# ChristophReich1996/Multi-StyleGAN

Measured on AMD Instinct MI355X. Metric: training images/sec (G+D step, 256^2, seq=3x2ch), higher is better.
Workload: dtype bf16

## Files before the change

include/msg_hip.h:

```cpp
#ifndef MSG_HIP_H
#define MSG_HIP_H

#ifdef __cplusplus
extern "C" {
#endif

enum { MSG_OK = 0, MSG_EINVAL = -1, MSG_EUNSUPPORTED = -2, MSG_ELAUNCH = -3 };
enum { MSG_F32 = 0, MSG_BF16 = 1, MSG_F16 = 2, MSG_F64 = 3, MSG_F32_SPLIT = 4 };

#define MSG_ABI_VERSION 5
int msg_abi_version(void);
const char* msg_build_arch(void);
const char* msg_strerror(int code);

int msg_upfirdn2d(const void* x, const float* fir, void* y, int dtype,
                  int major, int in_h, int in_w, int minor, int kh, int kw,
                  int up_x, int up_y, int down_x, int down_y,
                  int pad_x0, int pad_x1, int pad_y0, int pad_y1, void* stream);

int msg_upfirdn2d_pitched(const void* x, const float* fir, void* y, int dtype,
                          int major, int in_h, int in_w, int minor, int in_pitch, int kh, int kw,
                          int up_x, int up_y, int down_x, int down_y,
                          int pad_x0, int pad_x1, int pad_y0, int pad_y1, void* stream);

// ... 18 lines not shown
                                     int noise_batch, float alpha, float scale, unsigned char* mask, void* stream);

int msg_fused_bias_act(const void* x, const float* bias, const void* ref, void* y, int dtype,
                       long long size_x, int step_b, int size_b,
                       const float* noise, const float* noise_weight, int noise_batch, int pix,
                       int act, int grad, float alpha, float scale, void* stream);

long long msg_bias_act_backward_workspace(long long size_x, int step_b, int size_b, int has_noise);
int msg_bias_act_backward(const void* gy, const void* out, void* gx, int dtype,
                          long long size_x, int step_b, int size_b,
                          float* grad_bias, const float* noise, float* grad_noise_weight,
                          int noise_batch, int pix, float alpha, float scale,
                          float* ws, long long ws_floats, void* stream);
int msg_channel_sums(const void* x, float* sums, int dtype, long long size_x, int C, float* ws, long long ws_floats,
                     void* stream);
int msg_bias_act_backward_mask(const void* gy, const unsigned char* mask, int tile_m, int tile_n, void* gx, int dtype,
                               long long size_x, int size_b,
                               float* grad_bias, const float* noise, float* grad_noise_weight,
                               int noise_batch, int pix, float alpha, float scale,
                               float* ws, long long ws_floats, void* stream);
int msg_sum_rows(const float* part, float* out, long long rows, int cols, void* stream);
int msg_bias_act_backward_mask_head(const void* gy, const void* ghead, const float* whead, const float* style,
                                    float wscale, int n_head, const unsigned char* mask, int tile_m, int tile_n,
                                    void* gx, int dtype, long long size_x, int size_b,
                                    float* grad_bias, const float* noise, float* grad_noise_weight,
                                    int noise_batch, int pix, float alpha, float scale,
                                    float* ws, long long ws_floats, void* stream);

int msg_conv2d_fprop(const void* x, const void* w, const float* bias, void* y, int dtype,
                     int B, int IH, int IW, int Cx, int Ck, int OH, int OW, int N, int ldy,
                     int kh, int kw, int stride, int pad, int in_up, int pixel_shuffle,
                     long long w_batch_stride, void* stream);
int msg_conv2d_wgrad(const void* gy, const void* x, float* gw, int dtype,
                     int B, int IH, int IW, int Cx, int I, int OH, int OW, int ldgy, int O, int ldgw,
                     int kh, int kw, int stride, int pad, int pixel_shuffle,
                     int per_sample, int k_chunks, int oi_major, float gain,
                     float* ws, long long ws_floats, void* stream);
long long msg_conv2d_wgrad_workspace(int dtype, int B, int IH, int IW, int Cx, int I, int OH, int OW, int ldgy,
                                     int O, int ldgw, int kh, int kw, int stride, int pad, int pixel_shuffle,
                                     int per_sample, int k_chunks);

int msg_demod_coeff(const float* W, const float* s, float* d, int B, int O, int I, int taps,
                    float scale, float eps, void* stream);
int msg_scale_rows_cols(const float* base, const float* rowscale, const float* colscale, void* out,
                        int dtype, int B, int R, int T, int C, int Ck, float gain, void* stream);
int msg_modulate_weights(const float* base, const float* wsq, const float* style, void* out, float* d_out,
                         int dtype, int B, int R, int O, int T, int C, int Ck, float scale, float eps, void* stream);
int msg_modulate_backward(const float* gwk, const float* W, const float* s, const float* d, float* gW,
                          float* gs_part, int B, int O, int I, int taps, int ldg, int o_group,
                          float scale, void* stream);
int msg_scale_rows_cols2(const float* base, const float* row1, const float* col1, const float* row2, const float* col2,
                         void* out, int dtype, int B, int R, int T, int C, int Ck, float gain, void* stream);
int msg_modulate_backward2(const float* gwk, const float* W, const float* s, const float* d, const float* v,
                           float* gW, float* gs_part, int B, int O, int I, int taps, int ldg, int o_group,
                           float scale, void* stream);

int msg_relayout_weight(const float* w, void* fwd, void* dgrad, float* wsq, int dtype,
                        int O, int I, int T, int Ck, int Ok, int flip, int t_major, float gain, void* stream);

int msg_gather_taps(const void* x, void* y, int dtype, int B, int H, int W, int Cx, int C, int kh, int kw,
                    int pad, int Ko, void* stream);
int msg_fold_taps(const void* g, const void* add, void* gx, int dtype, int B, int H, int W, int Ko, int C, int kh, int kw,
                  int pad, int ldx, int ld_add, void* stream);

int msg_scaled_add(const void* a, const void* b, void* y, int dtype, long long n, float beta, float gain, void* stream);
int msg_rgb_skip_merge(const void* conv, int dtype, int ld, const float* bias, const float* skip, const float* fir,
                       float* out, int B, int C, int H, int W, void* stream);
int msg_rgb_skip_merge_backward(const float* g, void* g_conv, int dtype, int ld, float* g_skip, const float* fir,
                                int B, int C, int H, int W, void* stream);
int msg_gamma_merge(const void* a, const void* b, const float* gamma, void* y, int dtype, long long n, float gain, void* stream);
long long msg_gamma_merge_backward_workspace(void);
int msg_gamma_merge_backward(const void* gy, const void* a, const float* gamma, void* ga, void* gb, float* g_gamma, int dtype,
                             long long n, float gain, float* ws, void* stream);
int msg_scaled_add_rows(const void* a, const void* b, void* y, int dtype, long long rows, int cols,
                        long long lda, long long ldb, long long ldy, float beta, float gain, void* stream);

int msg_softmax_rows(const void* x, void* y, int dtype, long long rows, int cols, void* stream);
int msg_softmax_rows_backward(const void* y, const void* gy, void* gx, int dtype, long long rows, int cols,
                              void* stream);
int msg_softmax_rows_backward2(const void* y, const void* gy, const void* v, void* d_y, void* d_gy, int dtype,
                               long long rows, int cols, void* stream);

int msg_nonlocal_attention_supported(int B, int Nq, int Nk, int dk, int dv);
int msg_nonlocal_attention_fwd(const void* q, const void* k, const void* vt, void* o, float* lse, int dtype,
                               int B, int Nq, int Nk, int dk, int dv, void* stream);
int msg_maxpool2x2_fwd(const void* x, void* y, unsigned short* idx, int dtype, int B, int H, int W, int C, long long ldx,
                       void* stream);
int msg_maxpool2x2_bwd(const void* gy, const unsigned short* idx, void* gx, int dtype, int B, int H, int W, int C,
                       void* stream);
int msg_maxpool2x2_gather(const void* v, const unsigned short* idx, void* out, int dtype, int B, int H, int W, int C,
                          long long ldv, void* stream);

int msg_nonlocal_attention_bwd_splits(int B, int Nq, int Nk);
int msg_nonlocal_attention_bwd(const void* q, const void* qt, const void* k, const void* kt, const void* v,
                               const void* dO, const void* dOt, const void* o, const float* lse, float* delta,
                               void* dq, void* dk_out, void* dv_out, float* workspace, int dtype,
                               int B, int Nq, int Nk, int dk, int dv, void* stream);

int msg_affine_warp(const float* x, float* y, const float* angle_deg, float angle_const, const float* scale_xy,
                    const float* select_u, const float* p, int rot_prob, float cx, float cy, int padding,
                    int align_corners, int B, int C, int H, int W, int backward, void* workspace, void* stream);

long long msg_minibatch_stddev_workspace(int C, int H, int W, int groups, int dtype);
int msg_minibatch_stddev(const void* x, void* y, float* stat, float* workspace, int dtype,
                         int B, int C, int H, int W, int ldx, int ldy, int groups, float alpha, void* stream);
int msg_minibatch_stddev_backward(const void* x, const void* gy, const float* gstat, void* gx, int dtype,
                                  int B, int C, int H, int W, int ldx, int ldgy, int ldgx, int groups,
                                  float alpha, void* stream);

int msg_conv2d_fprop_act(const void* x, const void* w, void* y, int dtype,
                         int B, int IH, int IW, int Cx, int Ck, int OH, int OW, int N, int ldy,
                         int kh, int kw, int stride, int pad, long long w_batch_stride,
                         const float* act_bias, const float* noise, const float* noise_weight,
                         int noise_batch, float alpha, float scale, void* stream);
int msg_conv2d_fprop_act_mask(const void* x, const void* w, void* y, int dtype,
                              int B, int IH, int IW, int Cx, int Ck, int OH, int OW, int N, int ldy,
                              int kh, int kw, int stride, int pad, long long w_batch_stride,
                              const float* act_bias, const float* noise, const float* noise_weight,
                              int noise_batch, float alpha, float scale, unsigned char* mask, void* stream);

int msg_conv2d_fprop_residual(const void* x, const void* w, void* y, int dtype,
                              int B, int IH, int IW, int Cx, int Ck, int OH, int OW, int N, int ldy,
                              int kh, int kw, int stride, int pad, long long w_batch_stride,
                              const void* residual, int res_ld, float gain, void* stream);

int msg_conv2d_fprop_act_backward(const void* x, const void* w, void* y, int dtype,
                                  int B, int IH, int IW, int Cx, int Ck, int OH, int OW, int N, int ldy,
                                  int kh, int kw, int stride, int pad, long long w_batch_stride,
                                  const void* residual, int res_ld,
                                  const unsigned char* sign_mask, int mask_tile_m, int mask_tile_n,
                                  const void* sign_map, int sign_ld, float alpha, float scale,
                                  float* grad_bias, const float* noise, int noise_batch, float* grad_noise_weight,
                                  float* ws, long long ws_floats, void* stream);

int msg_act_pointwise_head(const void* x, const float* bias, const float* w, float* y, int dtype,
                           long long npix, int C, float wscale, float alpha, float scale, void* stream);
long long msg_act_pointwise_head_backward_workspace(long long npix, int C);
int msg_act_pointwise_head_backward(const void* x, const float* bias, const float* w, const float* gy, void* gx,
                                    float* grad_bias_and_w, int dtype, long long npix, int C, float wscale,
                                    float alpha, float scale, float* ws, long long ws_floats, void* stream);

int msg_linear_fprop(const float* x, const float* w, const float* bias, float* y, int M, int N, int K,
                     float gain, float bias_gain, void* stream);
int msg_linear_dgrad(const float* gy, const float* w, float* gx, int M, int N, int K, float gain, void* stream);
int msg_linear_wgrad(const float* gy, const float* x, float* gw, float* gb, int M, int N, int K,
                     float gain, float bias_gain, void* stream);

int msg_linear_grouped_fprop(const float* x, const int* slot, const float* const* w, const float* const* bias, float* y,
                             int G, int M, int N, int K, int L, float gain, float bias_gain, void* stream);
int msg_linear_grouped_dgrad(const float* gy, const float* const* w, float* gx, int G, int M, int N, int K, float gain,
                             void* stream);
int msg_linear_grouped_wgrad(const float* gy, const float* x, const int* slot, float* gw, float* gb, int G, int M, int N,
                             int K, int L, float gain, float bias_gain, void* stream);
int msg_linear_grouped_wgrad_ptrs(const float* gy, const float* x, const int* slot, float* const* gw, float* const* gb, int G,
                                  int M, int N, int K, int L, float gain, float bias_gain, void* stream);

enum {
    MSG_PLAN_REG = 0,
    MSG_PLAN_DMA = 1,
    MSG_PLAN_PP = 2,
    MSG_PLAN_ROW3 = 3,
    MSG_PLAN_ROW3N = 4,
    MSG_PLAN_THIN = 5,
    MSG_PLAN_UPCONV = 6,
    MSG_FPLAN_FIELDS = 5
};
int msg_conv2d_fprop_launch_plan(int dtype, int B, int IH, int IW, int Cx, int Ck, int OH, int OW, int N, int ldy,
// ... 56 lines not shown
```

multi_stylegan_amd/csrc/attention.hip:

```cpp
#include "msg_common.h"
#include <stdlib.h>

typedef __bf16 bf16v8 __attribute__((ext_vector_type(8)));

namespace {

template <typename T> struct Mma;
template <> struct Mma<bf16_t> {
    typedef bf16v8 Frag;
    static constexpr int KS = 16;
    static constexpr int PAD = 8;
    static constexpr int VEC = 8;
    static __device__ __forceinline__ Frag load(const bf16_t* row, int s, int h) {
        return *reinterpret_cast<const Frag*>(row + 16 * s + 8 * h);
    }
    static __device__ __forceinline__ f32x16 mma(Frag a, Frag b, f32x16 c) {
        return __builtin_amdgcn_mfma_f32_32x32x16_bf16(a, b, c, 0, 0, 0);
    }
    static __device__ __forceinline__ float dot(Frag a, Frag b) {
        float acc = 0.f;
#pragma unroll
        for (int j = 0; j < 8; ++j) acc = fmaf((float)a[j], (float)b[j], acc);
        return acc;
    }
    static __device__ __forceinline__ void store4(bf16_t* p, float a, float b, float c, float d) {
        uint2 v;
        v.x = (uint32_t)f2bf(a) | ((uint32_t)f2bf(b) << 16);
        v.y = (uint32_t)f2bf(c) | ((uint32_t)f2bf(d) << 16);
        *reinterpret_cast<uint2*>(p) = v;
    }
    static __device__ __forceinline__ Frag load_t(const bf16_t* tile, int pitch, int col, int s, int lane) {
        typedef short s16x4 __attribute__((ext_vector_type(4)));
        typedef short s16x8 __attribute__((ext_vector_type(8)));
        const int g = lane >> 4, q = (lane >> 2) & 3, pq = lane & 3;
        const int kb = 8 * (g >> 1), cb = 16 * (g & 1);
        s16x4 part[2];
#pragma unroll
        for (int half = 0; half < 2; ++half) {
            const bf16_t* pa = tile + (16 * s + kb + 4 * half + q) * pitch + col + cb + 4 * pq;
            part[half] = __builtin_amdgcn_ds_read_tr16_b64_v4i16((s16x4 __attribute__((address_space(3)))*)(pa));
        }
        return __builtin_bit_cast(Frag, (s16x8)__builtin_shufflevector(part[0], part[1], 0, 1, 2, 3, 4, 5, 6, 7));
    }
};
template <> struct Mma<float> {
    typedef float Frag;
    static constexpr int KS = 2;
    static constexpr int PAD = 4;
    static constexpr int VEC = 4;
    static __device__ __forceinline__ Frag load(const float* row, int s, int h) { return row[2 * s + h]; }
    static __device__ __forceinline__ f32x16 mma(Frag a, Frag b, f32x16 c) {
        return __builtin_amdgcn_mfma_f32_32x32x2f32(a, b, c, 0, 0, 0);
    }
    static __device__ __forceinline__ float dot(Frag a, Frag b) { return a * b; }
    static __device__ __forceinline__ void store4(float* p, float a, float b, float c, float d) {
        *reinterpret_cast<float4*>(p) = make_float4(a, b, c, d);
    }
    static __device__ __forceinline__ Frag load_t(const float* tile, int pitch, int col, int s, int lane) {
        return tile[(2 * s + (lane >> 5)) * pitch + col + (lane & 31)];
    }
};

template <typename T, int ROWS, int COLS, bool PF, int THREADS = 256>
struct Stager {
    static constexpr int VEC = 16 / sizeof(T), CPR = COLS / VEC, TOTAL = ROWS * CPR, N = (TOTAL + THREADS - 1) / THREADS;
    static_assert(COLS % VEC == 0, "tile rows are whole 16-byte vectors");
    uint4 r[PF ? N : 1];
    const T* src;
    long long pitch;
    __device__ __forceinline__ void load(const T* g, long long g_pitch, int tid) {
        if constexpr (!PF) { src = g; pitch = g_pitch; return; }
#pragma unroll
        for (int i = 0; i < N; ++i) {
            const int c = tid + THREADS * i;
            if (TOTAL % THREADS == 0 || c < TOTAL) {
                const int row = c / CPR, cc = c - row * CPR;
                r[PF ? i : 0] = *reinterpret_cast<const uint4*>(g + row * g_pitch + cc * VEC);
            }
        }
    }
    __device__ __forceinline__ void store(T* lds, int l_pitch, int tid) const {
#pragma unroll
        for (int i = 0; i < N; ++i) {
            const int c = tid + THREADS * i;
            if (TOTAL % THREADS == 0 || c < TOTAL) {
                const int row = c / CPR, cc = c - row * CPR;
                *reinterpret_cast<uint4*>(lds + row * l_pitch + cc * VEC) =
                    PF ? r[PF ? i : 0] : *reinterpret_cast<const uint4*>(src + row * pitch + cc * VEC);
            }
        }
    }
};

__device__ __forceinline__ f32x16 zero16() {
    f32x16 z;
#pragma unroll
    for (int i = 0; i < 16; ++i) z[i] = 0.f;
    return z;
}

__device__ __forceinline__ void wave_lds_fence() { asm volatile("s_waitcnt lgkmcnt(0)" ::: "memory"); }

template <typename T, int DK, int DV, bool PF>
__global__ __launch_bounds__(256) void nl_attn_fwd_kernel(const T* __restrict__ q, const T* __restrict__ k,
                                                         const T* __restrict__ vt, T* __restrict__ o,
                                                         float* __restrict__ lse, int Nq, int Nk) {
    using M = Mma<T>;
    constexpr int KB = 64, PAD = M::PAD, KSQ = DK / M::KS, KSP = KB / M::KS, NT = DV / 32;
    constexpr int KP = DK + PAD, VP = KB + PAD;
    __shared__ __attribute__((aligned(16))) T smem[KB * KP + DV * VP + 4 * 32 * VP];
    T* Ks = smem;
    T* Vs = Ks + KB * KP;
    T* Ps = Vs + DV * VP;
    const int tid = threadIdx.x, lane = tid & 63, wave = tid >> 6, r = lane & 31, h = lane >> 5;
    const int b = blockIdx.y, q0 = blockIdx.x * 128 + wave * 32;
    const T* qrow = q + ((long long)b * Nq + q0 + r) * DK;
    const T* kb = k + (long long)b * Nk * DK;
    const T* vtb = vt + (long long)b * DV * Nk;
    T* Pw = Ps + wave * 32 * VP;
    typename M::Frag qf[KSQ];
#pragma unroll
    for (int s = 0; s < KSQ; ++s) qf[s] = M::load(qrow, s, h);

    Stager<T, KB, DK, PF> kst;
    Stager<T, DV, KB, PF> vst;
    float m = -3.0e38f;
    kst.load(kb, DK, tid);
    for (int k0 = 0; k0 < Nk; k0 += KB) {
        __syncthreads();
        kst.store(Ks, KP, tid);
        __syncthreads();
        kst.load(kb + (long long)(k0 + KB < Nk ? k0 + KB : 0) * DK, DK, tid);
#pragma unroll
        for (int t = 0; t < KB / 32; ++t) {
            f32x16 acc = zero16();
#pragma unroll
            for (int s = 0; s < KSQ; ++s) acc = M::mma(M::load(Ks + (32 * t + r) * KP, s, h), qf[s], acc);
#pragma unroll
            for (int i = 0; i < 16; ++i) m = fmaxf(m, acc[i]);
        }
    }
    m = fmaxf(m, __shfl_xor(m, 32, 64));

    float l = 0.f;
    f32x16 oacc[NT];
#pragma unroll
    for (int n = 0; n < NT; ++n) oacc[n] = zero16();
    vst.load(vtb, Nk, tid);
    for (int k0 = 0; k0 < Nk; k0 += KB) {
        __syncthreads();
        kst.store(Ks, KP, tid);
        vst.store(Vs, VP, tid);
        __syncthreads();
        if (k0 + KB < Nk) {
            kst.load(kb + (long long)(k0 + KB) * DK, DK, tid);
            vst.load(vtb + k0 + KB, Nk, tid);
        }
#pragma unroll
        for (int t = 0; t < KB / 32; ++t) {
            f32x16 acc = zero16();
#pragma unroll
            for (int s = 0; s < KSQ; ++s) acc = M::mma(M::load(Ks + (32 * t + r) * KP, s, h), qf[s], acc);
#pragma unroll
            for (int g = 0; g < 4; ++g) {
                const float p0 = __expf(acc[4 * g] - m), p1 = __expf(acc[4 * g + 1] - m);
                const float p2 = __expf(acc[4 * g + 2] - m), p3 = __expf(acc[4 * g + 3] - m);
                l += (p0 + p1) + (p2 + p3);
                M::store4(Pw + r * VP + 32 * t + 8 * g + 4 * h, p0, p1, p2, p3);
            }
        }
        wave_lds_fence();
#pragma unroll
        for (int n = 0; n < NT; ++n)
#pragma unroll
            for (int s = 0; s < KSP; ++s)
                oacc[n] = M::mma(M::load(Vs + (32 * n + r) * VP, s, h), M::load(Pw + r * VP, s, h), oacc[n]);
    }
    l += __shfl_xor(l, 32, 64);
    const float inv = 1.f / l;
    if (h == 0) lse[(long long)b * Nq + q0 + r] = m + __logf(l);
    T* orow = o + ((long long)b * Nq + q0 + r) * DV;
#pragma unroll
    for (int n = 0; n < NT; ++n)
#pragma unroll
        for (int g = 0; g < 4; ++g)
            M::store4(orow + 32 * n + 8 * g + 4 * h, oacc[n][4 * g] * inv, oacc[n][4 * g + 1] * inv,
                      oacc[n][4 * g + 2] * inv, oacc[n][4 * g + 3] * inv);
}

template <typename T, int DK, int DV, bool PF>
__global__ __launch_bounds__(256) void nl_attn_bwd_q_kernel(const T* __restrict__ q, const T* __restrict__ k,
                                                           const T* __restrict__ kt, const T* __restrict__ v,
                                                           const T* __restrict__ dO, const T* __restrict__ o,
                                                           const float* __restrict__ lse,
                                                           float* __restrict__ delta, T* __restrict__ dq,
                                                           int Nq, int Nk) {
    using M = Mma<T>;
    constexpr int KB = 64, PAD = M::PAD, KSQ = DK / M::KS, KSV = DV / M::KS, KSP = KB / M::KS, MT = (DK + 31) / 32;
    constexpr int KP = DK + PAD, VP = DV + PAD, TP = KB + PAD;
    __shared__ __attribute__((aligned(16))) T smem[KB * KP + KB * VP + 32 * MT * TP + 4 * 32 * TP];
    T* Ks = smem;
    T* Vs = Ks + KB * KP;
    T* Kts = Vs + KB * VP;
    T* Ps = Kts + 32 * MT * TP;
    const int tid = threadIdx.x, lane = tid & 63, wave = tid >> 6, r = lane & 31, h = lane >> 5;
    const int b = blockIdx.y, q0 = blockIdx.x * 128 + wave * 32;
    const long long qi = (long long)b * Nq + q0 + r;
    const T* kb = k + (long long)b * Nk * DK;
    const T* ktb = kt + (long long)b * DK * Nk;
    const T* vb = v + (long long)b * Nk * DV;
    T* Pw = Ps + wave * 32 * TP;
    for (int c = tid; c < 32 * MT * TP; c += 256) Kts[c] = T(0);
    typename M::Frag qf[KSQ], dof[KSV];
#pragma unroll
    for (int s = 0; s < KSQ; ++s) qf[s] = M::load(q + qi * DK, s, h);
#pragma unroll
    for (int s = 0; s < KSV; ++s) dof[s] = M::load(dO + qi * DV, s, h);
    float Dl = 0.f;
#pragma unroll
    for (int s = 0; s < KSV; ++s) Dl += M::dot(dof[s], M::load(o + qi * DV, s, h));
    Dl += __shfl_xor(Dl, 32, 64);
    if (h == 0) delta[qi] = Dl;
    const float L = lse[qi];
    f32x16 dqacc[MT];
#pragma unroll
    for (int mt = 0; mt < MT; ++mt) dqacc[mt] = zero16();
    Stager<T, KB, DK, PF> kst;
    Stager<T, KB, DV, PF> vst;
    Stager<T, DK, KB, PF> ktst;
    kst.load(kb, DK, tid);
    vst.load(vb, DV, tid);
    ktst.load(ktb, Nk, tid);
    for (int k0 = 0; k0 < Nk; k0 += KB) {
        __syncthreads();
        kst.store(Ks, KP, tid);
        vst.store(Vs, VP, tid);
        ktst.store(Kts, TP, tid);
        __syncthreads();
        if (k0 + KB < Nk) {
            kst.load(kb + (long long)(k0 + KB) * DK, DK, tid);
            vst.load(vb + (long long)(k0 + KB) * DV, DV, tid);
            ktst.load(ktb + k0 + KB, Nk, tid);
        }
#pragma unroll
        for (int t = 0; t < KB / 32; ++t) {
            f32x16 sacc = zero16(), pacc = zero16();
#pragma unroll
            for (int s = 0; s < KSQ; ++s) sacc = M::mma(M::load(Ks + (32 * t + r) * KP, s, h), qf[s], sacc);
#pragma unroll
            for (int s = 0; s < KSV; ++s) pacc = M::mma(M::load(Vs + (32 * t + r) * VP, s, h), dof[s], pacc);
#pragma unroll
            for (int g = 0; g < 4; ++g) {
                float ds[4];
#pragma unroll
                for (int i = 0; i < 4; ++i) ds[i] = __expf(sacc[4 * g + i] - L) * (pacc[4 * g + i] - Dl);
                M::store4(Pw + r * TP + 32 * t + 8 * g + 4 * h, ds[0], ds[1], ds[2], ds[3]);
            }
        }
        wave_lds_fence();
#pragma unroll
        for (int mt = 0; mt < MT; ++mt)
#pragma unroll
            for (int s = 0; s < KSP; ++s)
                dqacc[mt] = M::mma(M::load(Kts + (32 * mt + r) * TP, s, h), M::load(Pw + r * TP, s, h), dqacc[mt]);
    }
    T* drow = dq + qi * DK;
#pragma unroll
    for (int mt = 0; mt < MT; ++mt)
#pragma unroll
        for (int g = 0; g < 4; ++g) {
            const int d0 = 32 * mt + 8 * g + 4 * h;
            if (d0 < DK)
                M::store4(drow + d0, dqacc[mt][4 * g], dqacc[mt][4 * g + 1], dqacc[mt][4 * g + 2], dqacc[mt][4 * g + 3]);
        }
}

template <typename T, int DK, int DV, int QB>
__global__ __launch_bounds__(512) void nl_attn_bwd_kv_kernel(const T* __restrict__ q, const T* __restrict__ qt,
                                                            const T* __restrict__ k, const T* __restrict__ v,
                                                            const T* __restrict__ dO, const T* __restrict__ dOt,
                                                            const float* __restrict__ lse,
                                                            const float* __restrict__ delta, T* __restrict__ dk,
                                                            T* __restrict__ dv, float* __restrict__ part, int Nq,
                                                            int Nk) {
    using M = Mma<T>;
    constexpr int PAD = M::PAD, KSQ = DK / M::KS, KSV = DV / M::KS, KSP = QB / M::KS, NT = DV / 32, MT = (DK + 31) / 32;
    constexpr int NH = NT / 2;
    static_assert(NT % 2 == 0 && MT <= 2, "the two waves of a key tile split the dv range and the dk tiles");
    constexpr int QP = DK + PAD, OP = DV + PAD, TP = QB + PAD;
    constexpr int STAT_T = (2 * QB * (int)sizeof(float)) / (int)sizeof(T);
    __shared__ __attribute__((aligned(16))) T smem[QB * QP + 64 + QB * OP + STAT_T + 2 * 4 * 32 * TP];
    T* Qs = smem;
    T* dOs = Qs + QB * QP + 64;
    float* Ls = reinterpret_cast<float*>(dOs + QB * OP);
    float* Ds = Ls + QB;
    T* Pts = reinterpret_cast<T*>(Ds + QB);
    T* dSts = Pts + 4 * 32 * TP;
    const int tid = threadIdx.x, lane = tid & 63, wave = tid >> 6, r = lane & 31, h = lane >> 5;
    const int kt = wave & 3, half = wave >> 2;
    const int b = blockIdx.y, key0 = blockIdx.x * 128 + kt * 32;
    const long long ki = (long long)b * Nk + key0 + r;
    const T* qb = q + (long long)b * Nq * DK;
    const T* dob = dO + (long long)b * Nq * DV;
    T* Ptw = Pts + kt * 32 * TP;
    T* dStw = dSts + kt * 32 * TP;
    typename M::Frag kf[KSQ], vf[KSV];
#pragma unroll
    for (int s = 0; s < KSQ; ++s) kf[s] = M::load(k + ki * DK, s, h);
#pragma unroll
    for (int s = 0; s < KSV; ++s) vf[s] = M::load(v + ki * DV, s, h);
    f32x16 dvacc[NH], dkacc = zero16();
#pragma unroll
    for (int n = 0; n < NH; ++n) dvacc[n] = zero16();
    const int q_per = Nq / gridDim.z, q_lo = blockIdx.z * q_per, q_hi = q_lo + q_per;
    for (int q0 = q_lo; q0 < q_hi; q0 += QB) {
        __syncthreads();
        Stager<T, QB, DK, false, 512> qst;
        Stager<T, QB, DV, false, 512> ost;
        qst.load(qb + (long long)q0 * DK, DK, tid);   qst.store(Qs, QP, tid);
        ost.load(dob + (long long)q0 * DV, DV, tid);  ost.store(dOs, OP, tid);
        if (tid < QB) Ls[tid] = lse[(long long)b * Nq + q0 + tid];
        else if (tid < 2 * QB) Ds[tid - QB] = delta[(long long)b * Nq + q0 + tid - QB];
        __syncthreads();
#pragma unroll
        for (int t = 0; t < QB / 32; ++t) {
            if ((t & 1) != half) continue;
            f32x16 sacc = zero16(), pacc = zero16();
#pragma unroll
            for (int s = 0; s < KSQ; ++s) sacc = M::mma(M::load(Qs + (32 * t + r) * QP, s, h), kf[s], sacc);
#pragma unroll
            for (int s = 0; s < KSV; ++s) pacc = M::mma(M::load(dOs + (32 * t + r) * OP, s, h), vf[s], pacc);
#pragma unroll
            for (int g = 0; g < 4; ++g) {
                const int qq = 32 * t + 8 * g + 4 * h;
                const float4 Lv = *reinterpret_cast<const float4*>(Ls + qq);
                const float4 Dv = *reinterpret_cast<const float4*>(Ds + qq);
                const float p0 = __expf(sacc[4 * g] - Lv.x), p1 = __expf(sacc[4 * g + 1] - Lv.y);
                const float p2 = __expf(sacc[4 * g + 2] - Lv.z), p3 = __expf(sacc[4 * g + 3] - Lv.w);
                M::store4(Ptw + r * TP + qq, p0, p1, p2, p3);
                M::store4(dStw + r * TP + qq, p0 * (pacc[4 * g] - Dv.x), p1 * (pacc[4 * g + 1] - Dv.y),
                          p2 * (pacc[4 * g + 2] - Dv.z), p3 * (pacc[4 * g + 3] - Dv.w));
            }
        }
        __syncthreads();
#pragma unroll
        for (int n = 0; n < NH; ++n)
#pragma unroll
            for (int s = 0; s < KSP; ++s)
                dvacc[n] = M::mma(M::load_t(dOs, OP, 32 * (half * NH + n), s, lane), M::load(Ptw + r * TP, s, h), dvacc[n]);
        if (half < MT) {
#pragma unroll
            for (int s = 0; s < KSP; ++s)
                dkacc = M::mma(M::load_t(Qs, QP, 32 * half, s, lane), M::load(dStw + r * TP, s, h), dkacc);
        }
    }
    if (gridDim.z > 1) {
        float* prow = part + ((long long)blockIdx.z * gridDim.y * Nk + ki) * (DV + DK);
#pragma unroll
        for (int n = 0; n < NH; ++n)
#pragma unroll
            for (int g = 0; g < 4; ++g)
                *reinterpret_cast<float4*>(prow + 32 * (half * NH + n) + 8 * g + 4 * h) =
                    make_float4(dvacc[n][4 * g], dvacc[n][4 * g + 1], dvacc[n][4 * g + 2], dvacc[n][4 * g + 3]);
        if (half < MT) {
#pragma unroll
            for (int g = 0; g < 4; ++g) {
                const int d0 = 32 * half + 8 * g + 4 * h;
                if (d0 < DK)
                    *reinterpret_cast<float4*>(prow + DV + d0) =
                        make_float4(dkacc[4 * g], dkacc[4 * g + 1], dkacc[4 * g + 2], dkacc[4 * g + 3]);
            }
        }
        return;
    }
    T* dvrow = dv + ki * DV;
#pragma unroll
    for (int n = 0; n < NH; ++n)
#pragma unroll
        for (int g = 0; g < 4; ++g)
            M::store4(dvrow + 32 * (half * NH + n) + 8 * g + 4 * h, dvacc[n][4 * g], dvacc[n][4 * g + 1],
                      dvacc[n][4 * g + 2], dvacc[n][4 * g + 3]);
    if (half < MT) {
        T* dkrow = dk + ki * DK;
#pragma unroll
        for (int g = 0; g < 4; ++g) {
            const int d0 = 32 * half + 8 * g + 4 * h;
            if (d0 < DK) M::store4(dkrow + d0, dkacc[4 * g], dkacc[4 * g + 1], dkacc[4 * g + 2], dkacc[4 * g + 3]);
        }
    }
}

template <typename T>
__global__ void nl_attn_reduce_kernel(const float* __restrict__ part, T* __restrict__ dk, T* __restrict__ dv,
                                      long long rows, int DK, int DV, int nsplit) {
    const long long i = (long long)blockIdx.x * blockDim.x + threadIdx.x;
    const int gpr = (DV + DK) / 4;
    if (i >= rows * gpr) return;
    const long long row = i / gpr;
    const int c = (int)(i - row * gpr) * 4;
    float4 acc = make_float4(0.f, 0.f, 0.f, 0.f);
    for (int z = 0; z < nsplit; ++z) {
        const float4 p = *reinterpret_cast<const float4*>(part + ((long long)z * rows + row) * (DV + DK) + c);
        acc.x += p.x; acc.y += p.y; acc.z += p.z; acc.w += p.w;
    }
    T* out = c < DV ? dv + row * DV + c : dk + row * DK + (c - DV);
    Mma<T>::store4(out, acc.x, acc.y, acc.z, acc.w);
}

int prefetch_mode() {
    static const int mode = msg_tunable("MSG_ATTN_PREFETCH", 0);
    return mode;
}

bool shapes_ok(int B, int Nq, int Nk, int dk, int dv) {
    return B > 0 && Nq > 0 && Nk > 0 && Nq % 128 == 0 && Nk % 128 == 0 && ((dk == 48 && dv == 192) || (dk == 16 && dv == 64));
}

template <typename T, int DK, int DV>
int launch_fwd(const void* q, const void* k, const void* vt, void* o, float* lse, int B, int Nq, int Nk, hipStream_t s) {
    if (prefetch_mode() & 1)
        hipLaunchKernelGGL((nl_attn_fwd_kernel<T, DK, DV, true>), dim3(Nq / 128, B), dim3(256), 0, s, (const T*)q,
                           (const T*)k, (const T*)vt, (T*)o, lse, Nq, Nk);
    else
        hipLaunchKernelGGL((nl_attn_fwd_kernel<T, DK, DV, false>), dim3(Nq / 128, B), dim3(256), 0, s, (const T*)q,
                           (const T*)k, (const T*)vt, (T*)o, lse, Nq, Nk);
    return MSG_CHECK_LAUNCH();
}

template <typename T, int DK, int DV>
int launch_bwd(const void* q, const void* qt, const void* k, const void* kt, const void* v, const void* dO,
               const void* dOt, const void* o, const float* lse, float* delta, void* dq, void* dk, void* dv,
               float* part, int nsplit, int B, int Nq, int Nk, hipStream_t s) {
    constexpr int QB = sizeof(T) == 2 ? 64 : 32;
    if (prefetch_mode() & 2)
        hipLaunchKernelGGL((nl_attn_bwd_q_kernel<T, DK, DV, true>), dim3(Nq / 128, B), dim3(256), 0, s, (const T*)q,
                           (const T*)k, (const T*)kt, (const T*)v, (const T*)dO, (const T*)o, lse, delta, (T*)dq, Nq, Nk);
    else
        hipLaunchKernelGGL((nl_attn_bwd_q_kernel<T, DK, DV, false>), dim3(Nq / 128, B), dim3(256), 0, s, (const T*)q,
                           (const T*)k, (const T*)kt, (const T*)v, (const T*)dO, (const T*)o, lse, delta, (T*)dq, Nq, Nk);
    if (hipGetLastError() != hipSuccess) return MSG_ELAUNCH;
    hipLaunchKernelGGL((nl_attn_bwd_kv_kernel<T, DK, DV, QB>), dim3(Nk / 128, B, nsplit), dim3(512), 0, s, (const T*)q,
                       (const T*)qt, (const T*)k, (const T*)v, (const T*)dO, (const T*)dOt, lse, delta, (T*)dk, (T*)dv,
                       part, Nq, Nk);
    if (nsplit > 1) {
        if (hipGetLastError() != hipSuccess) return MSG_ELAUNCH;
        const long long rows = (long long)B * Nk, groups = rows * ((DK + DV) / 4);
        hipLaunchKernelGGL((nl_attn_reduce_kernel<T>), dim3((unsigned)((groups + 255) / 256)), dim3(256), 0, s, part,
                           (T*)dk, (T*)dv, rows, DK, DV, nsplit);
    }
    return MSG_CHECK_LAUNCH();
}

}

extern "C" int msg_nonlocal_attention_supported(int B, int Nq, int Nk, int dk, int dv) {
    return shapes_ok(B, Nq, Nk, dk, dv) ? 1 : 0;
}

extern "C" int msg_nonlocal_attention_fwd(const void* q, const void* k, const void* vt, void* o, float* lse, int dtype,
                                          int B, int Nq, int Nk, int dk, int dv, void* stream) {
    if (!q || !k || !vt || !o || !lse) return MSG_EINVAL;
    if (!shapes_ok(B, Nq, Nk, dk, dv)) return MSG_EUNSUPPORTED;
    hipStream_t s = (hipStream_t)stream;
    if (dtype == MSG_BF16)
        return dk == 48 ? launch_fwd<bf16_t, 48, 192>(q, k, vt, o, lse, B, Nq, Nk, s)
                        : launch_fwd<bf16_t, 16, 64>(q, k, vt, o, lse, B, Nq, Nk, s);
    if (dtype == MSG_F32)
        return dk == 48 ? launch_fwd<float, 48, 192>(q, k, vt, o, lse, B, Nq, Nk, s)
                        : launch_fwd<float, 16, 64>(q, k, vt, o, lse, B, Nq, Nk, s);
    return MSG_EUNSUPPORTED;
}

extern "C" int msg_nonlocal_attention_bwd_splits(int B, int Nq, int Nk) {
    static const int forced = msg_tunable("MSG_ATTN_SPLITS", 0);
    if (forced > 0 && Nq % (forced * 128) == 0) return forced;
    int nsplit = 1;
    while (nsplit < 8 && (long long)B * (Nk / 128) * nsplit < 384 && (Nq / nsplit) % 128 == 0 && Nq / nsplit >= 512)
        nsplit *= 2;
    return nsplit;
}

extern "C" int msg_nonlocal_attention_bwd(const void* q, const void* qt, const void* k, const void* kt, const void* v,
                                          const void* dO, const void* dOt, const void* o, const float* lse,
                                          float* delta, void* dq, void* dk_out, void* dv_out, float* workspace,
                                          int dtype, int B, int Nq, int Nk, int dk, int dv, void* stream) {
    if (!q || !k || !kt || !v || !dO || !o || !lse || !delta || !dq || !dk_out || !dv_out) return MSG_EINVAL;
    if (!shapes_ok(B, Nq, Nk, dk, dv)) return MSG_EUNSUPPORTED;
    const int nsplit = msg_nonlocal_attention_bwd_splits(B, Nq, Nk);
    if (nsplit > 1 && !workspace) return MSG_EINVAL;
    float* part = workspace;
    hipStream_t s = (hipStream_t)stream;
    if (dtype == MSG_BF16)
        return dk == 48 ? launch_bwd<bf16_t, 48, 192>(q, qt, k, kt, v, dO, dOt, o, lse, delta, dq, dk_out, dv_out, part, nsplit, B, Nq, Nk, s)
                        : launch_bwd<bf16_t, 16, 64>(q, qt, k, kt, v, dO, dOt, o, lse, delta, dq, dk_out, dv_out, part, nsplit, B, Nq, Nk, s);
    if (dtype == MSG_F32)
        return dk == 48 ? launch_bwd<float, 48, 192>(q, qt, k, kt, v, dO, dOt, o, lse, delta, dq, dk_out, dv_out, part, nsplit, B, Nq, Nk, s)
                        : launch_bwd<float, 16, 64>(q, qt, k, kt, v, dO, dOt, o, lse, delta, dq, dk_out, dv_out, part, nsplit, B, Nq, Nk, s);
    return MSG_EUNSUPPORTED;
}
```

multi_stylegan_amd/op_static/attention.py:

```python

import torch
from torch.autograd import Function

from .. import _lib

def supported(q: torch.Tensor, k: torch.Tensor, v: torch.Tensor) -> bool:
    if not (q.is_cuda and q.dtype in (torch.float32, torch.bfloat16)
            and q.dtype == k.dtype == v.dtype and q.ndim == 3):
        return False
    return bool(_lib.lib().msg_nonlocal_attention_supported(q.shape[0], q.shape[1], k.shape[1], q.shape[2], v.shape[2]))


def composite(q: torch.Tensor, k: torch.Tensor, v: torch.Tensor) -> torch.Tensor:
    from .softmax import softmax_rows
    return torch.bmm(softmax_rows(torch.bmm(q, k.transpose(1, 2))), v)


class _NonLocalAttention(Function):
    @staticmethod
    def forward(ctx, q, k, v):
        dev = _lib.require_gpu(q, k, v)
        b, nq, dk = q.shape
        nk, dv = k.shape[1], v.shape[2]
        vt = v.transpose(1, 2).contiguous()
        o = torch.empty((b, nq, dv), dtype=q.dtype, device=dev)
        lse = torch.empty((b, nq), dtype=torch.float32, device=dev)
        flops = 2.0 * b * nq * nk * (2 * dk + dv)
        with _lib.on_device(dev), _lib.kernel_clock.span(('nl_attention_fwd', q.dtype), flops):
            code = _lib.lib().msg_nonlocal_attention_fwd(q.data_ptr(), k.data_ptr(), vt.data_ptr(), o.data_ptr(),
                                                         lse.data_ptr(), _lib.dtype_code(q), b, nq, nk, dk, dv,
                                                         _lib.stream_of(dev))
        _lib.check(code, "msg_nonlocal_attention_fwd")
        ctx.save_for_backward(q, k, v, o, lse)
        return o

    @staticmethod
    def backward(ctx, grad_o):
        q, k, v, o, lse = ctx.saved_tensors
        if torch.is_grad_enabled():
            with torch.enable_grad():
                qq, kk, vv = (t if t.requires_grad else t.detach().requires_grad_(True) for t in (q, k, v))
                return torch.autograd.grad(composite(qq, kk, vv), (qq, kk, vv), grad_o, create_graph=True)
        grad_o = grad_o.contiguous()
        dev = q.device
        b, nq, dk = q.shape
        nk, dv = k.shape[1], v.shape[2]
        delta = torch.empty((b, nq), dtype=torch.float32, device=dev)
        kt = k.transpose(1, 2).contiguous()
        dq, dkey, dval = torch.empty_like(q), torch.empty_like(k), torch.empty_like(v)
        splits = _lib.lib().msg_nonlocal_attention_bwd_splits(b, nq, nk)
        work = torch.empty(splits * b * nk * (dk + dv), dtype=torch.float32, device=dev) if splits > 1 else None
        flops = 2.0 * b * nq * nk * ((dk + dv + dk) + (dk + dv + dv + dk))
        with _lib.on_device(dev), _lib.kernel_clock.span(('nl_attention_bwd', q.dtype), flops):
            code = _lib.lib().msg_nonlocal_attention_bwd(
                q.data_ptr(), None, k.data_ptr(), kt.data_ptr(), v.data_ptr(), grad_o.data_ptr(),
                None, o.data_ptr(), lse.data_ptr(), delta.data_ptr(), dq.data_ptr(), dkey.data_ptr(),
                dval.data_ptr(),
                _lib.ptr(work), _lib.dtype_code(q), b, nq, nk, dk, dv, _lib.stream_of(dev))
        _lib.check(code, "msg_nonlocal_attention_bwd")
        return dq, dkey, dval


def non_local_attention(q: torch.Tensor, k: torch.Tensor, v: torch.Tensor) -> torch.Tensor:
    if supported(q, k, v):
        return _NonLocalAttention.apply(q.contiguous(), k.contiguous(), v.contiguous())
    return composite(q, k, v)
```

Before: 155.1.

## Fuse attention forward into single-pass online softmax and drop host transposes

The non-local attention forward kernel changes from a two-pass scheme (first a max pass over K, then the exp/PV pass) to a single-pass online softmax with rescaling. V is read in its natural layout through transposing LDS reads, so the host-side V and K transposes are removed from forward and backward. The backward dq kernel reads K transposed from LDS instead of staging a separate Kt tile. The dK/dV kernel gains register prefetch of Q, dO and stats, prefetch is on by default, and occupancy hints are added for bf16. These changes cut one full K sweep, two transpose copies and redundant loads, at the cost of conditional rescaling and more register pressure.

```diff
diff --git a/include/msg_hip.h b/include/msg_hip.h
--- a/include/msg_hip.h
+++ b/include/msg_hip.h
@@ -124,7 +124,7 @@
                                long long rows, int cols, void* stream);
 
 int msg_nonlocal_attention_supported(int B, int Nq, int Nk, int dk, int dv);
-int msg_nonlocal_attention_fwd(const void* q, const void* k, const void* vt, void* o, float* lse, int dtype,
+int msg_nonlocal_attention_fwd(const void* q, const void* k, const void* v, void* o, float* lse, int dtype,
                                int B, int Nq, int Nk, int dk, int dv, void* stream);
 int msg_maxpool2x2_fwd(const void* x, void* y, unsigned short* idx, int dtype, int B, int H, int W, int C, long long ldx,
                        void* stream);
diff --git a/multi_stylegan_amd/csrc/attention.hip b/multi_stylegan_amd/csrc/attention.hip
--- a/multi_stylegan_amd/csrc/attention.hip
+++ b/multi_stylegan_amd/csrc/attention.hip
@@ -1,7 +1,9 @@
 #include "msg_common.h"
 #include <stdlib.h>
+#include <utility>
 
 typedef __bf16 bf16v8 __attribute__((ext_vector_type(8)));
+typedef unsigned int u32x4 __attribute__((ext_vector_type(4)));
 
 namespace {
 
@@ -11,6 +13,7 @@
     static constexpr int KS = 16;
     static constexpr int PAD = 8;
     static constexpr int VEC = 8;
+    static constexpr int TPAD = 32;
     static __device__ __forceinline__ Frag load(const bf16_t* row, int s, int h) {
         return *reinterpret_cast<const Frag*>(row + 16 * s + 8 * h);
     }
@@ -48,6 +51,7 @@
     static constexpr int KS = 2;
     static constexpr int PAD = 4;
     static constexpr int VEC = 4;
+    static constexpr int TPAD = 4;
     static __device__ __forceinline__ Frag load(const float* row, int s, int h) { return row[2 * s + h]; }
     static __device__ __forceinline__ f32x16 mma(Frag a, Frag b, f32x16 c) {
         return __builtin_amdgcn_mfma_f32_32x32x2f32(a, b, c, 0, 0, 0);
@@ -65,30 +69,36 @@
 struct Stager {
     static constexpr int VEC = 16 / sizeof(T), CPR = COLS / VEC, TOTAL = ROWS * CPR, N = (TOTAL + THREADS - 1) / THREADS;
     static_assert(COLS % VEC == 0, "tile rows are whole 16-byte vectors");
-    uint4 r[PF ? N : 1];
+    u32x4 r[PF ? N : 1];
     const T* src;
     long long pitch;
+    template <int I> __device__ __forceinline__ void load_step(const T* g, long long g_pitch, int tid) {
+        const int c = tid + THREADS * I;
+        if (TOTAL % THREADS == 0 || c < TOTAL) {
+            const int row = c / CPR, cc = c - row * CPR;
+            r[PF ? I : 0] = *reinterpret_cast<const u32x4*>(g + row * g_pitch + cc * VEC);
+        }
+    }
+    template <int I> __device__ __forceinline__ void store_step(T* lds, int l_pitch, int tid) const {
+        const int c = tid + THREADS * I;
+        if (TOTAL % THREADS == 0 || c < TOTAL) {
+            const int row = c / CPR, cc = c - row * CPR;
+            *reinterpret_cast<u32x4*>(lds + row * l_pitch + cc * VEC) =
+                PF ? r[PF ? I : 0] : *reinterpret_cast<const u32x4*>(src + row * pitch + cc * VEC);
+        }
+    }
+    template <int... I> __device__ __forceinline__ void load_all(const T* g, long long p, int tid, std::integer_sequence<int, I...>) {
+        (load_step<I>(g, p, tid), ...);
+    }
+    template <int... I> __device__ __forceinline__ void store_all(T* lds, int p, int tid, std::integer_sequence<int, I...>) const {
+        (store_step<I>(lds, p, tid), ...);
+    }
     __device__ __forceinline__ void load(const T* g, long long g_pitch, int tid) {
         if constexpr (!PF) { src = g; pitch = g_pitch; return; }
-#pragma unroll
-        for (int i = 0; i < N; ++i) {
-            const int c = tid + THREADS * i;
-            if (TOTAL % THREADS == 0 || c < TOTAL) {
-                const int row = c / CPR, cc = c - row * CPR;
-                r[PF ? i : 0] = *reinterpret_cast<const uint4*>(g + row * g_pitch + cc * VEC);
-            }
-        }
+        load_all(g, g_pitch, tid, std::make_integer_sequence<int, N>());
     }
     __device__ __forceinline__ void store(T* lds, int l_pitch, int tid) const {
-#pragma unroll
-        for (int i = 0; i < N; ++i) {
-            const int c = tid + THREADS * i;
-            if (TOTAL % THREADS == 0 || c < TOTAL) {
-                const int row = c / CPR, cc = c - row * CPR;
-                *reinterpret_cast<uint4*>(lds + row * l_pitch + cc * VEC) =
-                    PF ? r[PF ? i : 0] : *reinterpret_cast<const uint4*>(src + row * pitch + cc * VEC);
-            }
-        }
+        store_all(lds, l_pitch, tid, std::make_integer_sequence<int, N>());
     }
 };
 
@@ -102,79 +112,76 @@
 __device__ __forceinline__ void wave_lds_fence() { asm volatile("s_waitcnt lgkmcnt(0)" ::: "memory"); }
 
 template <typename T, int DK, int DV, bool PF>
-__global__ __launch_bounds__(256) void nl_attn_fwd_kernel(const T* __restrict__ q, const T* __restrict__ k,
-                                                         const T* __restrict__ vt, T* __restrict__ o,
+__global__ __launch_bounds__(256, sizeof(T) == 2 ? 2 : 1) void nl_attn_fwd_kernel(const T* __restrict__ q, const T* __restrict__ k,
+                                                         const T* __restrict__ v, T* __restrict__ o,
                                                          float* __restrict__ lse, int Nq, int Nk) {
     using M = Mma<T>;
-    constexpr int KB = 64, PAD = M::PAD, KSQ = DK / M::KS, KSP = KB / M::KS, NT = DV / 32;
-    constexpr int KP = DK + PAD, VP = KB + PAD;
-    __shared__ __attribute__((aligned(16))) T smem[KB * KP + DV * VP + 4 * 32 * VP];
+    constexpr int KB = 64, PAD = M::PAD, KSQ = DK / M::KS, KSP = 32 / M::KS, NT = DV / 32;
+    constexpr int KP = DK + PAD, VP = DV + M::TPAD, PP = 32 + PAD;
+    __shared__ __attribute__((aligned(16))) T smem[KB * KP + KB * VP + 4 * 32 * PP];
     T* Ks = smem;
     T* Vs = Ks + KB * KP;
-    T* Ps = Vs + DV * VP;
+    T* Ps = Vs + KB * VP;
     const int tid = threadIdx.x, lane = tid & 63, wave = tid >> 6, r = lane & 31, h = lane >> 5;
     const int b = blockIdx.y, q0 = blockIdx.x * 128 + wave * 32;
     const T* qrow = q + ((long long)b * Nq + q0 + r) * DK;
     const T* kb = k + (long long)b * Nk * DK;
-    const T* vtb = vt + (long long)b * DV * Nk;
-    T* Pw = Ps + wave * 32 * VP;
+    const T* vb = v + (long long)b * Nk * DV;
+    T* Pw = Ps + wave * 32 * PP;
     typename M::Frag qf[KSQ];
 #pragma unroll
     for (int s = 0; s < KSQ; ++s) qf[s] = M::load(qrow, s, h);
 
     Stager<T, KB, DK, PF> kst;
-    Stager<T, DV, KB, PF> vst;
-    float m = -3.0e38f;
+    Stager<T, KB, DV, PF> vst;
+    float m = -3.0e38f, l = 0.f;
+    f32x16 oacc[NT];
+#pragma unroll
+    for (int n = 0; n < NT; ++n) oacc[n] = zero16();
     kst.load(kb, DK, tid);
+    vst.load(vb, DV, tid);
     for (int k0 = 0; k0 < Nk; k0 += KB) {
         __syncthreads();
         kst.store(Ks, KP, tid);
-        __syncthreads();
-        kst.load(kb + (long long)(k0 + KB < Nk ? k0 + KB : 0) * DK, DK, tid);
+        vst.store(Vs, VP, tid);
+        __syncthreads();
+        if (k0 + KB < Nk) {
+            kst.load(kb + (long long)(k0 + KB) * DK, DK, tid);
+            vst.load(vb + (long long)(k0 + KB) * DV, DV, tid);
+        }
 #pragma unroll
         for (int t = 0; t < KB / 32; ++t) {
             f32x16 acc = zero16();
 #pragma unroll
             for (int s = 0; s < KSQ; ++s) acc = M::mma(M::load(Ks + (32 * t + r) * KP, s, h), qf[s], acc);
-#pragma unroll
-            for (int i = 0; i < 16; ++i) m = fmaxf(m, acc[i]);
-        }
-    }
-    m = fmaxf(m, __shfl_xor(m, 32, 64));
-
-    float l = 0.f;
-    f32x16 oacc[NT];
-#pragma unroll
-    for (int n = 0; n < NT; ++n) oacc[n] = zero16();
-    vst.load(vtb, Nk, tid);
-    for (int k0 = 0; k0 < Nk; k0 += KB) {
-        __syncthreads();
-        kst.store(Ks, KP, tid);
-        vst.store(Vs, VP, tid);
-        __syncthreads();
-        if (k0 + KB < Nk) {
-            kst.load(kb + (long long)(k0 + KB) * DK, DK, tid);
-            vst.load(vtb + k0 + KB, Nk, tid);
-        }
-#pragma unroll
-        for (int t = 0; t < KB / 32; ++t) {
-            f32x16 acc = zero16();
-#pragma unroll
-            for (int s = 0; s < KSQ; ++s) acc = M::mma(M::load(Ks + (32 * t + r) * KP, s, h), qf[s], acc);
+            float bm = acc[0];
+#pragma unroll
+            for (int i = 1; i < 16; ++i) bm = fmaxf(bm, acc[i]);
+            bm = fmaxf(bm, __shfl_xor(bm, 32, 64));
+            if (__any(bm > m)) {
+                const float mn = fmaxf(m, bm), sc = __expf(m - mn);
+                m = mn;
+                l *= sc;
+#pragma unroll
+                for (int n = 0; n < NT; ++n)
+#pragma unroll
+                    for (int i = 0; i < 16; ++i) oacc[n][i] *= sc;
+            }
 #pragma unroll
             for (int g = 0; g < 4; ++g) {
                 const float p0 = __expf(acc[4 * g] - m), p1 = __expf(acc[4 * g + 1] - m);
                 const float p2 = __expf(acc[4 * g + 2] - m), p3 = __expf(acc[4 * g + 3] - m);
                 l += (p0 + p1) + (p2 + p3);
-                M::store4(Pw + r * VP + 32 * t + 8 * g + 4 * h, p0, p1, p2, p3);
+                M::store4(Pw + r * PP + 8 * g + 4 * h, p0, p1, p2, p3);
             }
-        }
-        wave_lds_fence();
-#pragma unroll
-        for (int n = 0; n < NT; ++n)
-#pragma unroll
-            for (int s = 0; s < KSP; ++s)
-                oacc[n] = M::mma(M::load(Vs + (32 * n + r) * VP, s, h), M::load(Pw + r * VP, s, h), oacc[n]);
+            wave_lds_fence();
+#pragma unroll
+            for (int n = 0; n < NT; ++n)
+#pragma unroll
+                for (int s = 0; s < KSP; ++s)
+                    oacc[n] = M::mma(M::load_t(Vs + 32 * t * VP, VP, 32 * n, s, lane), M::load(Pw + r * PP, s, h), oacc[n]);
+            wave_lds_fence();
+        }
     }
     l += __shfl_xor(l, 32, 64);
     const float inv = 1.f / l;
@@ -189,28 +196,25 @@
 }
 
 template <typename T, int DK, int DV, bool PF>
-__global__ __launch_bounds__(256) void nl_attn_bwd_q_kernel(const T* __restrict__ q, const T* __restrict__ k,
-                                                           const T* __restrict__ kt, const T* __restrict__ v,
-                                                           const T* __restrict__ dO, const T* __restrict__ o,
-                                                           const float* __restrict__ lse,
+__global__ __launch_bounds__(256, sizeof(T) == 2 ? 2 : 1) void nl_attn_bwd_q_kernel(const T* __restrict__ q, const T* __restrict__ k,
+                                                           const T* __restrict__ v, const T* __restrict__ dO,
+                                                           const T* __restrict__ o, const float* __restrict__ lse,
                                                            float* __restrict__ delta, T* __restrict__ dq,
                                                            int Nq, int Nk) {
     using M = Mma<T>;
     constexpr int KB = 64, PAD = M::PAD, KSQ = DK / M::KS, KSV = DV / M::KS, KSP = KB / M::KS, MT = (DK + 31) / 32;
     constexpr int KP = DK + PAD, VP = DV + PAD, TP = KB + PAD;
-    __shared__ __attribute__((aligned(16))) T smem[KB * KP + KB * VP + 32 * MT * TP + 4 * 32 * TP];
+    static_assert((KB - 1) * KP + 32 * MT <= KB * KP + KB * VP, "the transposing reads of K stay inside the array");
+    __shared__ __attribute__((aligned(16))) T smem[KB * KP + KB * VP + 4 * 32 * TP];
     T* Ks = smem;
     T* Vs = Ks + KB * KP;
-    T* Kts = Vs + KB * VP;
-    T* Ps = Kts + 32 * MT * TP;
+    T* Ps = Vs + KB * VP;
     const int tid = threadIdx.x, lane = tid & 63, wave = tid >> 6, r = lane & 31, h = lane >> 5;
     const int b = blockIdx.y, q0 = blockIdx.x * 128 + wave * 32;
     const long long qi = (long long)b * Nq + q0 + r;
     const T* kb = k + (long long)b * Nk * DK;
-    const T* ktb = kt + (long long)b * DK * Nk;
     const T* vb = v + (long long)b * Nk * DV;
     T* Pw = Ps + wave * 32 * TP;
-    for (int c = tid; c < 32 * MT * TP; c += 256) Kts[c] = T(0);
     typename M::Frag qf[KSQ], dof[KSV];
 #pragma unroll
     for (int s = 0; s < KSQ; ++s) qf[s] = M::load(q + qi * DK, s, h);
@@ -227,20 +231,16 @@
     for (int mt = 0; mt < MT; ++mt) dqacc[mt] = zero16();
     Stager<T, KB, DK, PF> kst;
     Stager<T, KB, DV, PF> vst;
-    Stager<T, DK, KB, PF> ktst;
     kst.load(kb, DK, tid);
     vst.load(vb, DV, tid);
-    ktst.load(ktb, Nk, tid);
     for (int k0 = 0; k0 < Nk; k0 += KB) {
         __syncthreads();
         kst.store(Ks, KP, tid);
         vst.store(Vs, VP, tid);
-        ktst.store(Kts, TP, tid);
         __syncthreads();
         if (k0 + KB < Nk) {
             kst.load(kb + (long long)(k0 + KB) * DK, DK, tid);
             vst.load(vb + (long long)(k0 + KB) * DV, DV, tid);
-            ktst.load(ktb + k0 + KB, Nk, tid);
         }
 #pragma unroll
         for (int t = 0; t < KB / 32; ++t) {
@@ -262,7 +262,7 @@
         for (int mt = 0; mt < MT; ++mt)
 #pragma unroll
             for (int s = 0; s < KSP; ++s)
-                dqacc[mt] = M::mma(M::load(Kts + (32 * mt + r) * TP, s, h), M::load(Pw + r * TP, s, h), dqacc[mt]);
+                dqacc[mt] = M::mma(M::load_t(Ks, KP, 32 * mt, s, lane), M::load(Pw + r * TP, s, h), dqacc[mt]);
     }
     T* drow = dq + qi * DK;
 #pragma unroll
@@ -275,7 +275,7 @@
         }
 }
 
-template <typename T, int DK, int DV, int QB>
+template <typename T, int DK, int DV, int QB, bool PF>
 __global__ __launch_bounds__(512) void nl_attn_bwd_kv_kernel(const T* __restrict__ q, const T* __restrict__ qt,
                                                             const T* __restrict__ k, const T* __restrict__ v,
                                                             const T* __restrict__ dO, const T* __restrict__ dOt,
@@ -313,15 +313,24 @@
 #pragma unroll
     for (int n = 0; n < NH; ++n) dvacc[n] = zero16();
     const int q_per = Nq / gridDim.z, q_lo = blockIdx.z * q_per, q_hi = q_lo + q_per;
+    Stager<T, QB, DK, PF, 512> qst;
+    Stager<T, QB, DV, PF, 512> ost;
+    const float* statp = tid < QB ? lse + (long long)b * Nq + tid : delta + (long long)b * Nq + (tid - QB);
+    float stat = 0.f;
+    qst.load(qb + (long long)q_lo * DK, DK, tid);
+    ost.load(dob + (long long)q_lo * DV, DV, tid);
+    if (tid < 2 * QB) stat = statp[q_lo];
     for (int q0 = q_lo; q0 < q_hi; q0 += QB) {
         __syncthreads();
-        Stager<T, QB, DK, false, 512> qst;
-        Stager<T, QB, DV, false, 512> ost;
-        qst.load(qb + (long long)q0 * DK, DK, tid);   qst.store(Qs, QP, tid);
-        ost.load(dob + (long long)q0 * DV, DV, tid);  ost.store(dOs, OP, tid);
-        if (tid < QB) Ls[tid] = lse[(long long)b * Nq + q0 + tid];
-        else if (tid < 2 * QB) Ds[tid - QB] = delta[(long long)b * Nq + q0 + tid - QB];
-        __syncthreads();
+        qst.store(Qs, QP, tid);
+        ost.store(dOs, OP, tid);
+        if (tid < 2 * QB) Ls[tid] = stat;
+        __syncthreads();
+        if (q0 + QB < q_hi) {
+            qst.load(qb + (long long)(q0 + QB) * DK, DK, tid);
+            ost.load(dob + (long long)(q0 + QB) * DV, DV, tid);
+            if (tid < 2 * QB) stat = statp[q0 + QB];
+        }
 #pragma unroll
         for (int t = 0; t < QB / 32; ++t) {
             if ((t & 1) != half) continue;
@@ -407,9 +416,9 @@
     Mma<T>::store4(out, acc.x, acc.y, acc.z, acc.w);
 }
 
-int prefetch_mode() {
-    static const int mode = msg_tunable("MSG_ATTN_PREFETCH", 0);
-    return mode;
+template <typename T> int prefetch_mode() {
+    static const int mode = msg_tunable("MSG_ATTN_PREFETCH", 0x37);
+    return sizeof(T) == 2 ? mode & 7 : (mode >> 4) & 7;
 }
 
 bool shapes_ok(int B, int Nq, int Nk, int dk, int dv) {
@@ -417,13 +426,13 @@
 }
 
 template <typename T, int DK, int DV>
-int launch_fwd(const void* q, const void* k, const void* vt, void* o, float* lse, int B, int Nq, int Nk, hipStream_t s) {
-    if (prefetch_mode() & 1)
+int launch_fwd(const void* q, const void* k, const void* v, void* o, float* lse, int B, int Nq, int Nk, hipStream_t s) {
+    if (prefetch_mode<T>() & 1)
         hipLaunchKernelGGL((nl_attn_fwd_kernel<T, DK, DV, true>), dim3(Nq / 128, B), dim3(256), 0, s, (const T*)q,
-                           (const T*)k, (const T*)vt, (T*)o, lse, Nq, Nk);
+                           (const T*)k, (const T*)v, (T*)o, lse, Nq, Nk);
     else
         hipLaunchKernelGGL((nl_attn_fwd_kernel<T, DK, DV, false>), dim3(Nq / 128, B), dim3(256), 0, s, (const T*)q,
-                           (const T*)k, (const T*)vt, (T*)o, lse, Nq, Nk);
+                           (const T*)k, (const T*)v, (T*)o, lse, Nq, Nk);
     return MSG_CHECK_LAUNCH();
 }
 
@@ -432,16 +441,21 @@
                const void* dOt, const void* o, const float* lse, float* delta, void* dq, void* dk, void* dv,
                float* part, int nsplit, int B, int Nq, int Nk, hipStream_t s) {
     constexpr int QB = sizeof(T) == 2 ? 64 : 32;
-    if (prefetch_mode() & 2)
+    if (prefetch_mode<T>() & 2)
         hipLaunchKernelGGL((nl_attn_bwd_q_kernel<T, DK, DV, true>), dim3(Nq / 128, B), dim3(256), 0, s, (const T*)q,
-                           (const T*)k, (const T*)kt, (const T*)v, (const T*)dO, (const T*)o, lse, delta, (T*)dq, Nq, Nk);
+                           (const T*)k, (const T*)v, (const T*)dO, (const T*)o, lse, delta, (T*)dq, Nq, Nk);
     else
         hipLaunchKernelGGL((nl_attn_bwd_q_kernel<T, DK, DV, false>), dim3(Nq / 128, B), dim3(256), 0, s, (const T*)q,
-                           (const T*)k, (const T*)kt, (const T*)v, (const T*)dO, (const T*)o, lse, delta, (T*)dq, Nq, Nk);
+                           (const T*)k, (const T*)v, (const T*)dO, (const T*)o, lse, delta, (T*)dq, Nq, Nk);
     if (hipGetLastError() != hipSuccess) return MSG_ELAUNCH;
-    hipLaunchKernelGGL((nl_attn_bwd_kv_kernel<T, DK, DV, QB>), dim3(Nk / 128, B, nsplit), dim3(512), 0, s, (const T*)q,
-                       (const T*)qt, (const T*)k, (const T*)v, (const T*)dO, (const T*)dOt, lse, delta, (T*)dk, (T*)dv,
-                       part, Nq, Nk);
+    if (prefetch_mode<T>() & 4)
+        hipLaunchKernelGGL((nl_attn_bwd_kv_kernel<T, DK, DV, QB, true>), dim3(Nk / 128, B, nsplit), dim3(512), 0, s,
+                           (const T*)q, (const T*)qt, (const T*)k, (const T*)v, (const T*)dO, (const T*)dOt, lse, delta,
+                           (T*)dk, (T*)dv, part, Nq, Nk);
+    else
+        hipLaunchKernelGGL((nl_attn_bwd_kv_kernel<T, DK, DV, QB, false>), dim3(Nk / 128, B, nsplit), dim3(512), 0, s,
+                           (const T*)q, (const T*)qt, (const T*)k, (const T*)v, (const T*)dO, (const T*)dOt, lse, delta,
+                           (T*)dk, (T*)dv, part, Nq, Nk);
     if (nsplit > 1) {
         if (hipGetLastError() != hipSuccess) return MSG_ELAUNCH;
         const long long rows = (long long)B * Nk, groups = rows * ((DK + DV) / 4);
@@ -457,17 +471,17 @@
     return shapes_ok(B, Nq, Nk, dk, dv) ? 1 : 0;
 }
 
-extern "C" int msg_nonlocal_attention_fwd(const void* q, const void* k, const void* vt, void* o, float* lse, int dtype,
+extern "C" int msg_nonlocal_attention_fwd(const void* q, const void* k, const void* v, void* o, float* lse, int dtype,
                                           int B, int Nq, int Nk, int dk, int dv, void* stream) {
-    if (!q || !k || !vt || !o || !lse) return MSG_EINVAL;
+    if (!q || !k || !v || !o || !lse) return MSG_EINVAL;
     if (!shapes_ok(B, Nq, Nk, dk, dv)) return MSG_EUNSUPPORTED;
     hipStream_t s = (hipStream_t)stream;
     if (dtype == MSG_BF16)
-        return dk == 48 ? launch_fwd<bf16_t, 48, 192>(q, k, vt, o, lse, B, Nq, Nk, s)
-                        : launch_fwd<bf16_t, 16, 64>(q, k, vt, o, lse, B, Nq, Nk, s);
+        return dk == 48 ? launch_fwd<bf16_t, 48, 192>(q, k, v, o, lse, B, Nq, Nk, s)
+                        : launch_fwd<bf16_t, 16, 64>(q, k, v, o, lse, B, Nq, Nk, s);
     if (dtype == MSG_F32)
-        return dk == 48 ? launch_fwd<float, 48, 192>(q, k, vt, o, lse, B, Nq, Nk, s)
-                        : launch_fwd<float, 16, 64>(q, k, vt, o, lse, B, Nq, Nk, s);
+        return dk == 48 ? launch_fwd<float, 48, 192>(q, k, v, o, lse, B, Nq, Nk, s)
+                        : launch_fwd<float, 16, 64>(q, k, v, o, lse, B, Nq, Nk, s);
     return MSG_EUNSUPPORTED;
 }
 
@@ -484,7 +498,7 @@
                                           const void* dO, const void* dOt, const void* o, const float* lse,
                                           float* delta, void* dq, void* dk_out, void* dv_out, float* workspace,
                                           int dtype, int B, int Nq, int Nk, int dk, int dv, void* stream) {
-    if (!q || !k || !kt || !v || !dO || !o || !lse || !delta || !dq || !dk_out || !dv_out) return MSG_EINVAL;
+    if (!q || !k || !v || !dO || !o || !lse || !delta || !dq || !dk_out || !dv_out) return MSG_EINVAL;
     if (!shapes_ok(B, Nq, Nk, dk, dv)) return MSG_EUNSUPPORTED;
     const int nsplit = msg_nonlocal_attention_bwd_splits(B, Nq, Nk);
     if (nsplit > 1 && !workspace) return MSG_EINVAL;
diff --git a/multi_stylegan_amd/op_static/attention.py b/multi_stylegan_amd/op_static/attention.py
--- a/multi_stylegan_amd/op_static/attention.py
+++ b/multi_stylegan_amd/op_static/attention.py
@@ -22,12 +22,11 @@
         dev = _lib.require_gpu(q, k, v)
         b, nq, dk = q.shape
         nk, dv = k.shape[1], v.shape[2]
-        vt = v.transpose(1, 2).contiguous()
         o = torch.empty((b, nq, dv), dtype=q.dtype, device=dev)
         lse = torch.empty((b, nq), dtype=torch.float32, device=dev)
         flops = 2.0 * b * nq * nk * (2 * dk + dv)
         with _lib.on_device(dev), _lib.kernel_clock.span(('nl_attention_fwd', q.dtype), flops):
-            code = _lib.lib().msg_nonlocal_attention_fwd(q.data_ptr(), k.data_ptr(), vt.data_ptr(), o.data_ptr(),
+            code = _lib.lib().msg_nonlocal_attention_fwd(q.data_ptr(), k.data_ptr(), v.data_ptr(), o.data_ptr(),
                                                          lse.data_ptr(), _lib.dtype_code(q), b, nq, nk, dk, dv,
                                                          _lib.stream_of(dev))
         _lib.check(code, "msg_nonlocal_attention_fwd")
@@ -46,14 +45,13 @@
         b, nq, dk = q.shape
         nk, dv = k.shape[1], v.shape[2]
         delta = torch.empty((b, nq), dtype=torch.float32, device=dev)
-        kt = k.transpose(1, 2).contiguous()
         dq, dkey, dval = torch.empty_like(q), torch.empty_like(k), torch.empty_like(v)
         splits = _lib.lib().msg_nonlocal_attention_bwd_splits(b, nq, nk)
         work = torch.empty(splits * b * nk * (dk + dv), dtype=torch.float32, device=dev) if splits > 1 else None
         flops = 2.0 * b * nq * nk * ((dk + dv + dk) + (dk + dv + dv + dk))
         with _lib.on_device(dev), _lib.kernel_clock.span(('nl_attention_bwd', q.dtype), flops):
             code = _lib.lib().msg_nonlocal_attention_bwd(
-                q.data_ptr(), None, k.data_ptr(), kt.data_ptr(), v.data_ptr(), grad_o.data_ptr(),
+                q.data_ptr(), None, k.data_ptr(), None, v.data_ptr(), grad_o.data_ptr(),
                 None, o.data_ptr(), lse.data_ptr(), delta.data_ptr(), dq.data_ptr(), dkey.data_ptr(),
                 dval.data_ptr(),
                 _lib.ptr(work), _lib.dtype_code(q), b, nq, nk, dk, dv, _lib.stream_of(dev))
```

Result: no change. 156.0, median of 4 (+0.6%).
